# deepalcoholic/mlcomp

Hardware: AMD Instinct MI355X
Metric: images/sec (whole node) ResNet-50 DAG train task (higher is better)
Workload: dtype bf16; 1 GPU; model=resnet50, global_batch=512, per_gpu_batch=512, image_size=224, parallelism=dp1, impl=native, optimizer=SGD momentum 0.9, wd 5e-5, fp32 master weights

## Files before the change

mlcomp_amd/ops/_lib.py:

```python
from __future__ import annotations

import ctypes as C
import os
import threading

import torch

_LIB = None
_LOCK = threading.Lock()

DETERMINISTIC = os.environ.get('MLC_DETERMINISTIC', '0') == '1'
DET_COPIES = max(32, int(os.environ.get('MLC_DET_COPIES', '4096')))

vp, i32, i64, f32, u32 = C.c_void_p, C.c_int, C.c_long, C.c_float, C.c_uint

_SIGS = {
    'mlc_conv_fwd': [vp, vp, vp, vp, vp] + [i32] * 12 + [vp, vp, vp],
    'mlc_conv_fwd_ld': [vp, vp, vp] + [i32] * 13 + [vp],
    'mlc_conv_dgrad': [vp] * 4 + [i32] * 12 + [vp] * 11 + [vp],
    'mlc_conv_dgrad_t': [vp] * 4 + [i32] * 12 + [vp] * 11 + [vp],
    'mlc_bilinear_up_fwd': [vp, vp] + [i32] * 6 + [vp],
    'mlc_bilinear_up_bwd': [vp, vp] + [i32] * 6 + [vp],
    'mlc_gn_relu_fwd': [vp, vp, vp, vp, vp] + [i32] * 4 + [f32, vp],
    'mlc_gn_relu_bwd': [vp] * 7 + [i32] * 4 + [f32, vp],
    'mlc_conv_tr_fwd': [vp] * 5 + [i32] * 12 + [vp],
    'mlc_wt_transpose': [vp, i32, i64, vp],
    'mlc_conv_wgrad': [vp, vp, vp] + [i32] * 14 + [vp, i64, vp, vp, vp],
    'mlc_conv_wgrad_native': [vp, vp, vp] + [i32] * 14 + [vp, i64, vp, vp, vp],
    'mlc_gemm_f32out': [vp, vp, vp, vp] + [i32] * 11 + [vp],
    'mlc_gemm_bf16out': [vp, vp, vp] + [i32] * 8 + [vp],
    'mlc_gemm256_nt': [vp, vp, vp, vp] + [i32] * 6 + [vp, i32, vp, vp, i32, i32, vp],
    'mlc_g256_dense': [vp, vp, vp] + [i32] * 7 + [vp, i32, vp, vp, vp, i32, vp],
    'mlc_gemm256_tn': [vp, vp, vp] + [i32] * 8 + [vp],
    'mlc_conv256_fwd': [vp] * 5 + [i32] * 13 + [vp],
    'mlc_augment': [vp, vp, vp, vp] + [i32] * 7 + [vp],
    'mlc_gemm_bf16_ex': [vp, vp, vp] + [i32] * 8 + [vp, i32, vp, vp, vp, vp, i64, vp],
    'mlc_gemm_bf16_ex_native': [vp, vp, vp] + [i32] * 8 + [vp, i32, vp, vp, vp, vp, i64, vp],
    'mlc_ln_fwd': [vp] * 8 + [i32, i32, f32, f32, f32, vp, u32, u32, vp],
    'mlc_ln_bwd': [vp] * 10 + [i32, i32, f32, f32, vp, u32, u32, vp],
    'mlc_ln_finalize_many': [vp, i32, i32, vp],
    'mlc_embed_bwd': [vp] * 7 + [i32] * 4 + [vp],
    'mlc_softmax_fwd': [vp] * 4 + [i64, i32, i32, f32, f32, vp, u32, vp],
    'mlc_softmax_bwd': [vp] * 3 + [i64, i32, f32, f32, vp, u32, vp],
    'mlc_linear_wgrad_bias': [vp] * 4 + [i32] * 7 + [vp, i64, vp],
    'mlc_linear_wgrad_bias_native': [vp] * 4 + [i32] * 7 + [vp, i64, vp],
    'mlc_blaslt_mode': [i32],
    'mlc_blaslt_choices': [vp, i32],
    'mlc_upcat_fwd': [vp, vp, vp] + [i32] * 5 + [vp],
    'mlc_upcat_bwd': [vp, vp, vp] + [i32] * 5 + [vp],
    'mlc_seg_head_fwd': [vp] * 6 + [i64, i32, i32, vp],
    'mlc_seg_head_bwd': [vp] * 8 + [i64, i32, i32, f32, f32, f32, vp],
    'mlc_attn_fwd': [vp] * 4 + [i32, i32, i32, f32, f32, vp, u32, vp],
    'mlc_attn_bwd': [vp] * 5 + [i32, i32, i32, f32, f32, vp, u32, vp],
    'mlc_flash_fwd': [vp] * 4 + [i32] * 4 + [f32, f32, vp, u32, vp],
    'mlc_flash_bwd': [vp] * 7 + [i32] * 4 + [f32, f32, vp, u32, vp],
    'mlc_flash_fwd_masked': [vp] * 4 + [i32] * 4 + [f32, f32, vp, u32, i32, vp, i64, i64, vp],
    'mlc_flash_bwd_masked': [vp] * 7 + [i32] * 4 + [f32, f32, vp, u32, i32, vp, i64, i64, vp],
    'mlc_flash_bwd128': [i32],
    'mlc_colsum_acc': [vp, vp, vp, i32, i32, vp],
    'mlc_dropout': [vp, vp, i64, f32, vp, u32, vp],
    'mlc_bn_stat_copies': [],
    'mlc_set_deterministic': [i32, i32],
    'mlc_get_stat_copies': [],
    'mlc_get_deterministic': [],
    'mlc_gemm_config': [i32],
    'mlc_gemm_get_set': [i32, i32],
    'mlc_bn_get_set': [i32, i32],
    'mlc_bn_finalize': [vp, vp, i32] + [vp] * 8 + [i64, i32, f32, f32, vp],
    'mlc_bn_fwd_apply': [vp] * 5 + [i64, i32, i32, vp],
    'mlc_bn_fwd_apply2': [vp] * 7 + [i64, i32, i32, vp],
    'mlc_bn_bwd_reduce': [vp] * 5 + [i64, i32, vp],
    'mlc_bn_bwd_finalize': [vp] * 6 + [i64, i32, vp],
    'mlc_bn_fwd_fused': [vp] * 5 + [i32] + [vp] * 10 + [i64, i32, f32, f32, i32, vp],
    'mlc_bn_bwd_fused': [vp] * 5 + [i32] + [vp] * 6 + [i64, i32, vp],
    'mlc_bnact_fused': [vp] * 5 + [i32] + [vp] * 10 + [i64, i32, f32, f32, i32, f32, vp, i64, vp, i32, vp, i64, vp],
    'mlc_bn_bwd_apply': [vp] * 7 + [i64, i32, vp],
    'mlc_conv1x1_bn_bwd': [vp] * 18 + [i64, i32, i32, vp],
    'mlc_conv1x1_bn_bwd_ok': [i32, i32],
    'mlc_conv1x1_bwd_get_set': [i32, i32],
    'mlc_maxpool_fwd': [vp, vp, vp] + [i32] * 9 + [vp],
    'mlc_maxpool_bwd': [vp, vp, vp] + [i32] * 9 + [vp],
    'mlc_stem_pool_fwd': [vp] * 6 + [i32] * 4 + [vp],
    'mlc_stem_pool_bwd_reduce_pooled': [vp] * 5 + [i32] * 4 + [vp],
    'mlc_stem_pool_bwd_reduce': [vp] * 5 + [i32] * 4 + [vp],
    'mlc_stem_pool_bwd_apply': [vp] * 6 + [i32] * 4 + [vp],
    'mlc_stem_s2d': [vp, vp] + [i32] * 5 + [vp],
    'mlc_stem_conv_fwd': [vp] * 5 + [i32] * 3 + [vp],
    'mlc_avgpool_fwd': [vp, vp, i32, i32, i32, vp],
    'mlc_avgpool_bwd': [vp, vp, vp, i32, i32, i32, vp],
    'mlc_avgpool2d_fwd': [vp, vp] + [i32] * 10 + [vp],
    'mlc_avgpool2d_bwd': [vp, vp, vp] + [i32] * 10 + [vp],
    'mlc_adaptive_avg_fwd': [vp, vp] + [i32] * 6 + [vp],
    'mlc_adaptive_avg_bwd': [vp, vp] + [i32] * 6 + [vp],
    'mlc_softmax_ce': [vp] * 5 + [i32, i32, i32, f32, f32, vp],
    'mlc_colsum': [vp, vp, i32, i32, vp],
    'mlc_nchw_to_nhwc': [vp, vp, i32, i32, i32, i32, vp],
    'mlc_cast_f32_bf16': [vp, vp, i64, vp],
    'mlc_sgd': [vp] * 5 + [i64, i64, i64, f32, f32, f32, i32, i32, vp],
    'mlc_adam': [vp] * 6 + [i64, i64, i64, f32, f32, f32, f32, i32, vp],
    'mlc_sqnorm': [vp, i64, vp, f32, vp],
    'mlc_opt_config': [i32, i32],
    'mlc_gconv_wb_elems': [i32] * 6,
    'mlc_gconv_fwd': [vp] * 6 + [i32] * 13 + [vp],
    'mlc_gconv_dgrad': [vp] * 4 + [i32] * 13 + [vp],
    'mlc_gconv_wgrad': [vp] * 3 + [i32] * 14 + [vp],
    'mlc_dwconv_fwd': [vp] * 5 + [i32] * 11 + [vp],
    'mlc_dwconv_dgrad': [vp] * 3 + [i32] * 11 + [vp],
    'mlc_dwconv_wgrad': [vp] * 4 + [i32] * 12 + [vp],
    'mlc_bn_stats': [vp, vp, vp, i64, i32, vp],
    'mlc_zero4': [vp, i64, vp, i64, vp, i64, vp, i64, vp],
    'mlc_bn_stats_ld': [vp, vp, vp, i64, i32, i32, i64, vp],
    'mlc_bnact_apply': [vp] * 7 + [i64, i32, i32, f32, vp, i64, vp],
    'mlc_bnact_bwd_reduce': [vp] * 10 + [i64, i32, i32, f32, vp, i64, i64, vp],
    'mlc_bnact_bwd': [vp] * 12 + [i64] + [vp] * 5 + [i64, i32, i32, f32, vp, i64, vp, i64, i64, vp, i32, vp],
    'mlc_bnact_bwd_apply': [vp] * 12 + [i64, i32, i32, f32, vp, i64, vp, i64, i64, vp, i32, vp],
    'mlc_act_fwd': [vp, vp, i64, i32, f32, vp],
    'mlc_act_bwd': [vp] * 4 + [i64, i32, f32, vp],
    'mlc_chscale_fwd': [vp] * 4 + [i32, i64, i32, i32, vp],
    'mlc_chscale_bwd': [vp] * 8 + [i32] * 3 + [vp],
    'mlc_conv_fwd_ex': [vp] * 4 + [i32] * 13 + [vp],
    'mlc_conv_wgrad_bias': [vp] * 4 + [i32] * 13 + [vp, i64, vp],
    'mlc_temporal_unfold': [vp, vp] + [i32] * 9 + [vp],
    'mlc_temporal_fold': [vp, vp, vp] + [i32] * 9 + [vp],
    'mlc_counters_owner': [i32],
    'mlc_counters_release': [i32],
    'mlc_counters_in_use': [],
    'mlc_comm_unique_id_bytes': [],
    'mlc_comm_get_unique_id': [vp],
    'mlc_comm_init': [vp, i32, i32, i32, i32, vp],
    'mlc_comm_async_error': [vp],
    'mlc_comm_abort': [vp],
    'mlc_comm_error_string': [i32],
    'mlc_comm_last_error': [vp],
    'mlc_comm_set_timeout': [i64],
    'mlc_comm_destroy': [vp],
    'mlc_allreduce': [vp, vp, vp, i64, i32, i32, vp],
    'mlc_broadcast': [vp, vp, vp, i64, i32, i32, vp],
    'mlc_reduce_scatter': [vp, vp, vp, i64, i32, i32, vp],
    'mlc_allgather': [vp, vp, vp, i64, i32, vp],
    'mlc_alltoall': [vp, vp, vp, i64, i32, i32, i32, vp],
}
_RESTYPE = {'mlc_comm_init': vp, 'mlc_gconv_wb_elems': C.c_long, 'mlc_counters_owner': None,
            'mlc_counters_release': C.c_long, 'mlc_counters_in_use': C.c_long,
            'mlc_comm_error_string': C.c_char_p, 'mlc_comm_last_error': C.c_char_p, 'mlc_comm_set_timeout': None}


def lib_path():
    from mlcomp_amd.build import KERNEL_LIB
    return os.environ.get('MLC_KERNEL_LIB') or KERNEL_LIB


def load():
    global _LIB
    if _LIB is not None:
        return _LIB
    with _LOCK:
        if _LIB is not None:
            return _LIB
        path = lib_path()
        if not os.path.exists(path):
            from mlcomp_amd.build import build_kernels
            build_kernels()
        lib = C.CDLL(path)
        for name, args in _SIGS.items():
            fn = getattr(lib, name)
            fn.argtypes = args
            fn.restype = _RESTYPE.get(name, C.c_int)
        for key, env in ((1, 'MLC_SPLIT_TARGET'), (2, 'MLC_SPLIT_TARGET_MAT'), (3, 'MLC_GEMM_BIG'),
                         (4, 'MLC_GEMM_BIG_MIN'), (5, 'MLC_GEMM_SINGLE_STAGE'), (6, 'MLC_SPLITK_FUSED'),
                         (9, 'MLC_SPLIT_TARGET_DENSE'), (12, 'MLC_DENSE_SPLIT_TARGET'), (13, 'MLC_SINGLE_STAGE_KT'),
                         (15, 'MLC_GEMM_PERSIST_NBUF'), (16, 'MLC_GEMM_PERSIST_KT')):
            if os.environ.get(env):
                lib.mlc_gemm_get_set(key, int(os.environ[env]))
        for key, env in ((0, 'MLC_BN_UNROLL'), (1, 'MLC_BN_BLOCKS')):
            if os.environ.get(env):
                lib.mlc_bn_get_set(key, int(os.environ[env]))
        if os.environ.get('MLC_FUSE_1X1_BLOCKS'):
            lib.mlc_conv1x1_bwd_get_set(0, int(os.environ['MLC_FUSE_1X1_BLOCKS']))
        if DETERMINISTIC:
            lib.mlc_set_deterministic(1, DET_COPIES)
            torch.use_deterministic_algorithms(True, warn_only=True)
        _LIB = lib
    return _LIB


def available() -> bool:
    return torch.cuda.is_available()


def stream():
    return C.c_void_p(torch.cuda.current_stream().cuda_stream)


def ptr(t):
    if t is None:
        return None
    return C.c_void_p(t.data_ptr())


def call(name, *args):
    rc = getattr(load(), name)(*args)
    if rc == -2 and DETERMINISTIC:
        raise RuntimeError(f'{name}: deterministic mode needs more partial-sum copies than '
                           f'MLC_DET_COPIES={DET_COPIES} (one per contributing block; raise it)')
    if rc != 0:
        raise RuntimeError(f'{name} failed (rc={rc}); check shape constraints '
                           f'(channels % 8 == 0) or HIP error')
    return rc
```

mlcomp_amd/ops/functional.py:

```python
from __future__ import annotations

from typing import Optional, Tuple

import contextlib
import math
import os
import threading

import torch
import torch.nn.functional as F

from . import _lib


def _cuda(t):
    return t is not None and t.is_cuda


def conv_out_hw(H, W, KH, KW, stride, pad, dil):
    ph, pw = (pad, pad) if isinstance(pad, int) else tuple(pad)
    Ho = (H + 2 * ph - dil * (KH - 1) - 1) // stride + 1
    Wo = (W + 2 * pw - dil * (KW - 1) - 1) // stride + 1
    return Ho, Wo


def pack_pad(pad) -> int:
    if isinstance(pad, int):
        return pad
    ph, pw = (int(v) for v in pad)
    return ph if ph == pw else (1 << 30) | (pw << 15) | ph


def bn_relu_input(x: torch.Tensor, in_affine) -> torch.Tensor:
    sc, sh = in_affine
    return torch.relu(x.float() * sc + sh).to(torch.bfloat16)


def conv2d_fwd(x: torch.Tensor, w: torch.Tensor, stride=1, pad=0, dil=1,
               stats: Optional[Tuple[torch.Tensor, torch.Tensor]] = None,
               out: Optional[torch.Tensor] = None, in_affine=None) -> torch.Tensor:
    N, H, W, C = x.shape
    Co, KH, KW, Ci = w.shape
    assert Ci == C, (w.shape, x.shape)
    Ho, Wo = conv_out_hw(H, W, KH, KW, stride, pad, dil)
    if _cuda(x):
        y = out if out is not None else torch.empty(N, Ho, Wo, Co, device=x.device, dtype=torch.bfloat16)
        ldy = rows_ld(y)
        if ldy != Co:
            assert ldy is not None and stats is None and in_affine is None, (y.shape, y.stride())
            _lib.call('mlc_conv_fwd_ld', _lib.ptr(x), _lib.ptr(w), _lib.ptr(y), ldy, N, H, W, C, Co, KH, KW, stride,
                      pack_pad(pad), dil, Ho, Wo, _lib.stream())
            return y
        s1, s2 = (stats if stats is not None else (None, None))
        sc, sh = in_affine if in_affine is not None else (None, None)
        _lib.call('mlc_conv_fwd', _lib.ptr(x), _lib.ptr(w), _lib.ptr(y), _lib.ptr(s1), _lib.ptr(s2),
                  N, H, W, C, Co, KH, KW, stride, pack_pad(pad), dil, Ho, Wo, _lib.ptr(sc), _lib.ptr(sh), _lib.stream())
        return y
    if in_affine is not None:
        x = bn_relu_input(x, in_affine)
    yf = F.conv2d(x.permute(0, 3, 1, 2).float(), w.permute(0, 3, 1, 2).float(), None, stride, pad, dil)
    if stats is not None:
        stats[0][:Co].add_(yf.sum(dim=(0, 2, 3)))
        stats[1][:Co].add_((yf * yf).sum(dim=(0, 2, 3)))
    y = yf.permute(0, 2, 3, 1).to(torch.bfloat16).contiguous()
    if out is not None:
        out.copy_(y)
        return out
    return y


def conv_transpose2d_fwd(x: torch.Tensor, w: torch.Tensor, out_hw, stride=2, pad=1, dil=1,
                         stats: Optional[Tuple[torch.Tensor, torch.Tensor]] = None) -> torch.Tensor:
    N, Hi, Wi, Cin = x.shape
    Cw, KH, KW, Cout = w.shape
    assert Cw == Cin, (w.shape, x.shape)
    Ho, Wo = out_hw
    assert conv_out_hw(Ho, Wo, KH, KW, stride, pad, dil) == (Hi, Wi), (out_hw, x.shape)
    if _cuda(x):
        y = torch.empty(N, Ho, Wo, Cout, device=x.device, dtype=torch.bfloat16)
        s1, s2 = (stats if stats is not None else (None, None))
        _lib.call('mlc_conv_tr_fwd', _lib.ptr(x), _lib.ptr(w), _lib.ptr(y), _lib.ptr(s1), _lib.ptr(s2),
                  N, Hi, Wi, Cin, Cout, KH, KW, stride, pack_pad(pad), dil, Ho, Wo, _lib.stream())
        return y
    oph = Ho - ((Hi - 1) * stride - 2 * pad + dil * (KH - 1) + 1)
    opw = Wo - ((Wi - 1) * stride - 2 * pad + dil * (KW - 1) + 1)
    yf = F.conv_transpose2d(x.permute(0, 3, 1, 2).float(), w.permute(0, 3, 1, 2).float(), None, stride, pad,
                            (oph, opw), 1, dil)
    if stats is not None:
        stats[0][:Cout].add_(yf.sum(dim=(0, 2, 3)))
        stats[1][:Cout].add_((yf * yf).sum(dim=(0, 2, 3)))
    return yf.permute(0, 2, 3, 1).to(torch.bfloat16).contiguous()


class BnBwdSpec:

    def __init__(self, mask, ys, affine=None):
        assert 1 <= len(ys) <= 2
        assert affine is None or (mask is None and len(affine) == len(ys))
        self.mask = mask
        self.ys = list(ys)
        self.affine = list(affine) if affine is not None else None


def wt_flip_transpose(w: torch.Tensor) -> torch.Tensor:
    return w.flip(1, 2).permute(3, 1, 2, 0).contiguous()


def dgrad_as_fwd_conv(KH, KW, stride, pad, dil) -> bool:
    return stride == 1 and pad <= dil * (KH - 1) and dil * (KH - 1) - pad == dil * (KW - 1) - pad


class WtTable:

    def __init__(self):
        self.slots = []
        self.views = []
        self.buf = None
        self.desc = None
        self.blocks = 0
        self._srcs = None

    def add(self, slot) -> int:
        self.slots.append(slot)
        return len(self.slots) - 1

    def __getitem__(self, i) -> torch.Tensor:
        return self.views[i]

    @staticmethod
    def _dims(shape):
        return tuple(shape) if len(shape) == 4 else (shape[0], 1, 1, shape[1])

    def finalize(self, device):
        if not self.slots:
            return
        total = sum((s.numel + 63) // 64 * 64 for s in self.slots)
        self.buf = torch.zeros(total, device=device, dtype=torch.bfloat16)
        off = 0
        for s in self.slots:
            Co, KH, KW, Ci = self._dims(s.shape)
            v = self.buf[off:off + s.numel]
            self.views.append(v.view(Ci, KH, KW, Co) if len(s.shape) == 4 else v.view(Ci, Co))
            off += (s.numel + 63) // 64 * 64
        if self.buf.is_cuda:
            self._build()

    def _build(self):
        rows, blk = [], 0
        for s, v in zip(self.slots, self.views):
            Co, KH, KW, Ci = self._dims(s.shape)
            rows.append([s.bf16.data_ptr(), v.data_ptr(), Co, KH * KW, Ci, blk])
            blk += KH * KW * ((Co + 63) // 64) * ((Ci + 63) // 64)
        self.desc = torch.tensor(rows, dtype=torch.int64).to(self.buf.device)
        self.blocks = blk
        self._srcs = [r[0] for r in rows]

    def refresh(self):
        if self.buf is None:
            return
        if not self.buf.is_cuda:
            for s, v in zip(self.slots, self.views):
                v.copy_(wt_flip_transpose(s.bf16) if s.bf16.dim() == 4 else s.bf16.t())
            return
        if self._srcs != [s.bf16.data_ptr() for s in self.slots]:
            self._build()
        _lib.call('mlc_wt_transpose', _lib.ptr(self.desc), len(self.slots), self.blocks, _lib.stream())


def conv2d_dgrad(dy: torch.Tensor, w: torch.Tensor, x_shape, stride=1, pad=0, dil=1,
                 addend: Optional[torch.Tensor] = None, out: Optional[torch.Tensor] = None,
                 bn: Optional[BnBwdSpec] = None, wt: Optional[torch.Tensor] = None) -> torch.Tensor:
    N, H, W, C = x_shape
    Co, KH, KW, Ci = w.shape
    _, Ho, Wo, _ = dy.shape
    if _cuda(dy):
        dx = out if out is not None else torch.empty(N, H, W, C, device=dy.device, dtype=torch.bfloat16)
        b = [None] * 11
        if bn is not None:
            b[0] = bn.mask
            for k, (yk, mk, sk) in enumerate(bn.ys):
                b[1 + 3 * k:4 + 3 * k] = [yk, mk, sk]
            for k, (ak, hk) in enumerate(bn.affine or []):
                b[7 + 2 * k:9 + 2 * k] = [ak, hk]
        if wt is not None:
            assert tuple(wt.shape) == (Ci, KH, KW, Co), (wt.shape, w.shape)
            _lib.call('mlc_conv_dgrad_t', _lib.ptr(dy), _lib.ptr(wt), _lib.ptr(dx), _lib.ptr(addend), N, H, W,
                      C, Co, KH, KW, stride, pack_pad(pad), dil, Ho, Wo, *[_lib.ptr(t) for t in b], _lib.stream())
            return dx
        _lib.call('mlc_conv_dgrad', _lib.ptr(dy), _lib.ptr(w), _lib.ptr(dx), _lib.ptr(addend), N, H, W, C,
                  Co, KH, KW, stride, pack_pad(pad), dil, Ho, Wo, *[_lib.ptr(t) for t in b], _lib.stream())
        return dx
    if wt is not None and isinstance(pad, int) and dgrad_as_fwd_conv(KH, KW, stride, pad, dil):
        dxf = F.conv2d(dy.permute(0, 3, 1, 2).float(), wt.permute(0, 3, 1, 2).float(), None, 1,
                       dil * (KH - 1) - pad, dil)
    else:
        if wt is not None:
            w = wt_flip_transpose(wt)
        dxf = torch.nn.grad.conv2d_input((N, C, H, W), w.permute(0, 3, 1, 2).float(),
                                         dy.permute(0, 3, 1, 2).float(), stride, pad, dil)
    dxf = dxf.permute(0, 2, 3, 1)
    if addend is not None:
        dxf = dxf + addend.float()
    if bn is not None:
        if bn.mask is not None:
            dxf = dxf * (bn.mask.float() > 0)
        elif bn.affine is not None:
            q = sum(yk.float() * ak + hk for (yk, _, _), (ak, hk) in zip(bn.ys, bn.affine))
            dxf = dxf * (q > 0)
        d = dxf.to(torch.bfloat16).float().reshape(-1, C)
        for yk, mk, sk in bn.ys:
            sv = sk.view(NSTAT, 2, C)
            sv[0, 0] += d.sum(0)
            sv[0, 1] += (d * (yk.float().reshape(-1, C) - mk)).sum(0)
    dx = dxf.to(torch.bfloat16).contiguous()
    if out is not None:
        out.copy_(dx)
        return out
    return dx


_USE_SLAB = os.environ.get('MLC_WGRAD_SLAB', '1') != '0'
_SLAB = {}
_SLAB_OLD = []


_ROLE = threading.local()


def register_side_stream(stream) -> None:
    """Kept for callers of the old API: the workspace role is now explicit (side_role)."""


@contextlib.contextmanager
def side_stream(stream):
    prev = getattr(_ROLE, 'side', False)
    _ROLE.side = True
    try:
        with torch.cuda.stream(stream):
            yield
    finally:
        _ROLE.side = prev


class CounterLease:
    _next = 0

    def __init__(self, device):
        CounterLease._next += 1
        self.owner = CounterLease._next
        self.device = torch.device(device)

    def release(self):
        if self.owner and torch.cuda.is_available():
            from . import _lib
            with torch.cuda.device(self.device):
                _lib.load().mlc_counters_release(self.owner)
        self.owner = 0

    def __del__(self):
        try:
            self.release()
        except Exception:
            pass


@contextlib.contextmanager
def capture_scope(store: dict):
    prev = getattr(_ROLE, 'capture', None)
    _ROLE.capture = store
    lease = None
    if torch.cuda.is_available():
        from . import _lib
        lease = store.setdefault('__counter_lease__', CounterLease(torch.cuda.current_device()))
        _lib.load().mlc_counters_owner(lease.owner)
    try:
        yield
    finally:
        _ROLE.capture = prev
        if lease is not None:
            _lib.load().mlc_counters_owner(0)


def workspace_key(device) -> str:
    device = torch.device(device)
    if device.type == 'cuda' and getattr(_ROLE, 'side', False):
        return f'{device}/side'
    return str(device)


def workspace_store(pool: dict) -> dict:
    cap = getattr(_ROLE, 'capture', None)
    if cap is not None and torch.cuda.is_available() and torch.cuda.is_current_stream_capturing():
        return cap.setdefault(id(pool), {})
    return pool


def slab_workspace(device, n: int) -> torch.Tensor:
    key = workspace_key(device)
    store = workspace_store(_SLAB)
    buf = store.get(key)
    if buf is None or buf.numel() < n:
        if buf is not None:
            _SLAB_OLD.append(buf)
        buf = torch.empty(max(n, 1 << 20), device=device, dtype=torch.float32)
        store[key] = buf
    return buf


def conv2d_wgrad(dy: torch.Tensor, x: torch.Tensor, w_shape, stride=1, pad=0, dil=1,
                 out: Optional[torch.Tensor] = None, accumulate=False, in_affine=None,
                 slab: Optional[bool] = None) -> torch.Tensor:
    Co, KH, KW, Ci = w_shape
    N, H, W, C = x.shape
    _, Ho, Wo, _ = dy.shape
    if _cuda(dy):
        dw = out if out is not None else torch.empty(Co, KH, KW, Ci, device=dy.device, dtype=torch.float32)
        use = _USE_SLAB if slab is None else slab
        ws = slab_workspace(dy.device, min(32 * Co * KH * KW * Ci, 64 << 20)) if use else None
        sc, sh = in_affine if in_affine is not None else (None, None)
        _lib.call('mlc_conv_wgrad', _lib.ptr(dy), _lib.ptr(x), _lib.ptr(dw), N, H, W, C, Co, KH, KW,
                  stride, pack_pad(pad), dil, Ho, Wo, 0, int(accumulate), _lib.ptr(ws),
                  ws.numel() if ws is not None else 0, _lib.ptr(sc), _lib.ptr(sh), _lib.stream())
        return dw
    if in_affine is not None:
        x = bn_relu_input(x, in_affine)
    dwf = torch.nn.grad.conv2d_weight(x.permute(0, 3, 1, 2).float(), (Co, Ci, KH, KW),
                                      dy.permute(0, 3, 1, 2).float(), stride, pad, dil)
    dwf = dwf.permute(0, 2, 3, 1)
    if out is not None:
        if accumulate:
            out.add_(dwf.reshape(out.shape))
        else:
            out.copy_(dwf.reshape(out.shape))
        return out
    return dwf.contiguous()


NSTAT = _lib.DET_COPIES if _lib.DETERMINISTIC else 32


def stat_buffers(C, device):
    b = torch.zeros(2, NSTAT * C, device=device, dtype=torch.float32)
    return b[0], b[1]


BN_FUSED = os.environ.get('MLC_BN_FUSED', '1') == '1'


def _bn_fused_ok(C, ncopy):
    return BN_FUSED and not _lib.DETERMINISTIC and C % 8 == 0 and C >= 8 and 1 <= ncopy <= 64


def bn_fwd_apply(y, res, s1, s2, gamma, beta, save_mean, save_invstd, run_mean, run_var,
                 eps=1e-5, momentum=0.1, relu=True, out=None, scale=None, shift=None,
                 res_affine=None, apply=True):
    rows = y.numel() // y.shape[-1]
    C = y.shape[-1]
    ncopy = s1.numel() // C
    if _cuda(y):
        if scale is None:
            scale = torch.empty(2, C, device=y.device, dtype=torch.float32)
            scale, shift = scale[0], scale[1]
        if apply and _bn_fused_ok(C, ncopy):
            z = out if out is not None else torch.empty_like(y)
            rs, rh = res_affine if res_affine is not None else (None, None)
            _lib.call('mlc_bn_fwd_fused', _lib.ptr(y), _lib.ptr(res), _lib.ptr(z), _lib.ptr(s1), _lib.ptr(s2), ncopy,
                      _lib.ptr(gamma), _lib.ptr(beta), _lib.ptr(save_mean), _lib.ptr(save_invstd), _lib.ptr(scale),
                      _lib.ptr(shift), _lib.ptr(run_mean), _lib.ptr(run_var), _lib.ptr(rs), _lib.ptr(rh), rows, C,
                      float(eps), float(momentum), int(relu), _lib.stream())
            return z
# ... 1025 lines not shown
```

mlcomp_amd/ops/layers.py:

```python
from __future__ import annotations

import os
from typing import List, Optional

import torch
import torch.nn as nn

from . import functional as Fn
from .arena import ParamArena, Slot

DGRAD_FIRST_ENV = os.environ.get('MLC_DGRAD_FIRST')


class Workspace:

    def __init__(self):
        self._req: List[tuple] = []
        self.buf = None
        self.views = {}

    def request(self, key, n):
        self._req.append((key, int(n)))
        return key

    def finalize(self, device):
        total = sum((n + 63) // 64 * 64 for _, n in self._req) or 64
        self.buf = torch.zeros(total, device=device, dtype=torch.float32)
        off = 0
        for key, n in self._req:
            self.views[key] = self.buf[off:off + n]
            off += (n + 63) // 64 * 64

    def __getitem__(self, key):
        return self.views[key]

    def zero(self):
        self.buf.zero_()


class NativeContext:

    def __init__(self):
        self.arena = ParamArena()
        self.ws = Workspace()
        self.anchor = None
        self.training = True
        self.device = None
        self.grad_prezeroed = False
        self.wgrad_stream = None
        self.wt = Fn.WtTable() if os.environ.get('MLC_DGRAD_WT', '1') == '1' else None
        self.wt_stale = False
        self.wgrad_lag = int(os.environ.get('MLC_WGRAD_LAG', '0') or 0)
        self.wgrad_defer = False
        self._pending_wgrad = []
        self.dgrad_first = DGRAD_FIRST_ENV == '1'
        self.wgrad_slab = os.environ.get('MLC_WGRAD_SLAB', '1') != '0'

    def default_wgrad_slab(self, on: bool):
        if os.environ.get('MLC_WGRAD_SLAB') is None:
            self.wgrad_slab = on

    def default_dgrad_first(self, on: bool):
        if DGRAD_FIRST_ENV is None:
            self.dgrad_first = on

    def finalize(self, device):
        self.device = torch.device(device)
        self.arena.finalize(device)
        self.ws.finalize(device)
        if self.wt is not None:
            self.wt.finalize(self.device)
        self.anchor = torch.zeros(1, device=device, requires_grad=True)
        self.arena.flush = self.flush_wgrad
        if self.device.type == 'cuda' and os.environ.get('MLC_WGRAD_STREAM', '1') in ('1', '2'):
            self.wgrad_stream = torch.cuda.Stream(self.device)
        self.default_wgrad_defer(False)

    def default_wgrad_defer(self, on: bool):
        env = os.environ.get('MLC_WGRAD_DEFER')
        self.wgrad_defer = (env == '1') if env is not None else on
        self.arena.grad_streams = [self.wgrad_stream] if (self.wgrad_defer and self.wgrad_stream) else []

    def flush_wgrad(self):
        if self.wgrad_defer and self.wgrad_stream is not None:
            cur = torch.cuda.current_stream(self.device)
            if cur != self.wgrad_stream:
                cur.wait_stream(self.wgrad_stream)
        self.join_wgrads(0)

    def default_wgrad_lag(self, n: int):
        if os.environ.get('MLC_WGRAD_LAG') is None:
            self.wgrad_lag = n

    def lag_wgrad(self, ev, keep, slots):
        self._pending_wgrad.append((ev, keep, slots))
        self.join_wgrads(self.wgrad_lag)

    def join_wgrads(self, keep_last: int):
        q = self._pending_wgrad
        while len(q) > keep_last:
            ev, _keep, slots = q.pop(0)
            cur = torch.cuda.current_stream(self.device)
            if cur != self.wgrad_stream:
                cur.wait_event(ev)
            for s in (slots if isinstance(slots, (list, tuple)) else (slots,)):
                self.arena.mark_ready(s)

    def refresh_wt(self):
        if self.wt is not None and self.training:
            self.wt.refresh()
        self.wt_stale = False


def flatten_bn_buffers(units) -> Optional[torch.Tensor]:
    units = [u for u in units if getattr(u, 'run_mean', None) is not None]
    if not units:
        return None
    flat = torch.empty(sum(2 * u.run_mean.numel() for u in units), device=units[0].run_mean.device)
    off = 0
    for u in units:
        C = u.run_mean.numel()
        flat[off:off + C].copy_(u.run_mean)
        flat[off + C:off + 2 * C].copy_(u.run_var)
        u.run_mean, u.run_var = flat[off:off + C], flat[off + C:off + 2 * C]
        off += 2 * C
    return flat


class ConvBN:

    def __init__(self, ctx: NativeContext, name: str, conv: nn.Conv2d, bn: nn.BatchNorm2d,
                 act: bool, cin_pad: Optional[int] = None, s2d: bool = False):
        assert conv.groups == 1, 'native ConvBN supports groups=1'
        self.ctx = ctx
        self.name = name
        Co, Ci, KH, KW = conv.weight.shape
        self.cin = Ci
        self.cin_p = cin_pad or Ci
        self.Co = Co
        self.k = (KH, KW)
        self.stride = conv.stride[0]
        self.pad = conv.padding[0]
        self.dil = conv.dilation[0]
        self.s2d = s2d
        if s2d:
            assert (KH, KW, self.stride, self.pad, self.dil) == (7, 7, 2, 3, 1) and Ci <= 3, \
                's2d stem needs a 7x7/2 pad-3 conv over <= 3 channels'
            self.k, self.stride, self.pad, self.cin_p = (4, 4), 1, 0, 16
            KH = KW = 4
        self.act = act
        self.eps = bn.eps
        self.momentum = bn.momentum if bn.momentum is not None else 0.1
        self.w = ctx.arena.weight(f'{name}.conv.weight', (Co, KH, KW, self.cin_p))
        self.wt_idx = None
        if ctx.wt is not None and not s2d:
            self.wt_idx = ctx.wt.add(self.w)
        self.gamma = ctx.arena.vector(f'{name}.bn.weight', (Co,))
        self.beta = ctx.arena.vector(f'{name}.bn.bias', (Co,))
        self._src = (conv, bn)
        self.k_s1 = ctx.ws.request(f'{name}.s1', Fn.NSTAT * Co)
        self.k_s2 = ctx.ws.request(f'{name}.s2', Fn.NSTAT * Co)
        self.k_bw = ctx.ws.request(f'{name}.bwd', Fn.NSTAT * 2 * Co)

    def load_from_torch(self):
        conv, bn = self._src
        dev = self.ctx.device
        if self.s2d:
            w = Fn.stem_w_to_s2d(conv.weight.detach().cpu())
            self._gmask = (Fn.stem_w_to_s2d(torch.ones(self.Co, self.cin, 7, 7)) != 0).float().to(dev)
        else:
            w = conv.weight.detach().permute(0, 2, 3, 1).float()
            if self.cin_p != self.cin:
                w = torch.nn.functional.pad(w, (0, self.cin_p - self.cin))
        self.w.master.copy_(w.to(dev))
        self.gamma.master.copy_(bn.weight.detach().to(dev))
        self.beta.master.copy_(bn.bias.detach().to(dev))
        self.run_mean = bn.running_mean.detach().clone().float().to(dev)
        self.run_var = bn.running_var.detach().clone().float().to(dev)
        Co = self.Co
        b = torch.zeros(7, Co, device=dev)
        self.save_mean, self.save_invstd, self.scale, self.shift = b[0], b[1], b[2], b[3]
        self.coef = b[4:7].reshape(-1)

    def export_to_torch(self):
        conv, bn = self._src
        if self.s2d:
            w = Fn.stem_w_from_s2d(self.w.master.detach().float().cpu(), self.cin)
        else:
            w = self.w.master[..., :self.cin].permute(0, 3, 1, 2).contiguous()
        conv.weight.data.copy_(w.to(conv.weight.device))
        bn.weight.data.copy_(self.gamma.master.to(bn.weight.device))
        bn.bias.data.copy_(self.beta.master.to(bn.bias.device))
        bn.running_mean.copy_(self.run_mean.to(bn.running_mean.device))
        bn.running_var.copy_(self.run_var.to(bn.running_var.device))

    def __call__(self, x, res=None):
        return _ConvBNFn.apply(x, res, self.ctx.anchor, self)

    def fwd(self, x, res=None, defer=False, in_affine=None):
        ws = self.ctx.ws
        if self.s2d and x.shape[-1] != 16:
            x = Fn.stem_s2d(x, 3)
        raff = None
        if isinstance(res, tuple):
            res, rs, rh = res
            raff = (rs, rh)
        if not self.ctx.training:
            y = self._conv(x, None, in_affine)
            torch.rsqrt(self.run_var + self.eps, out=self.scale).mul_(self.gamma.master)
            torch.sub(self.beta.master, self.run_mean * self.scale, out=self.shift)
            if defer:
                return None, (x, y, None)
            z = Fn.bn_apply(y, res, self.scale, self.shift, self.act, res_affine=raff)
            return z, (x, y, z)
        s1, s2 = ws[self.k_s1], ws[self.k_s2]
        self.ctx.wt_stale = True
        y = self._conv(x, (s1, s2), in_affine)
        training = self.ctx.training
        z = Fn.bn_fwd_apply(y, res, s1, s2, self.gamma.master, self.beta.master, self.save_mean,
                            self.save_invstd, self.run_mean if training else None,
                            self.run_var if training else None, self.eps, self.momentum, self.act,
                            scale=self.scale, shift=self.shift, res_affine=raff, apply=not defer)
        return z, (x, y, z)

    def _conv(self, x, stats, in_affine=None):
        if self.s2d and in_affine is None:
            return Fn.stem_conv_fwd(x, self.w.bf16, stats=stats)
        return Fn.conv2d_fwd(x, self.w.bf16, self.stride, self.pad, self.dil, stats=stats, in_affine=in_affine)

    def _dgrad(self, dy, x_shape, addend=None, out=None, bn=None):
        wt = None
        if self.wt_idx is not None:
            if self.ctx.wt_stale:
                raise RuntimeError('transposed filters are stale: the model must call '
                                   'ctx.refresh_wt() after its training forward pass')
            wt = self.ctx.wt[self.wt_idx]
        return Fn.conv2d_dgrad(dy, self.w.bf16, x_shape, self.stride, self.pad, self.dil,
                               addend=addend, out=out, bn=bn, wt=wt)

    def dgrad_covers_all(self) -> bool:
        return True

    def bn_target(self, rec):
        x, y, z = rec
        return (y, self.save_mean, self.ctx.ws[self.k_bw])

    def wgrad(self, dy, x, in_affine=None):
        Fn.conv2d_wgrad(dy, x, self.w.shape, self.stride, self.pad, self.dil, out=self.w.grad,
                        accumulate=self.ctx.grad_prezeroed, in_affine=in_affine, slab=self.ctx.wgrad_slab)
        if self.s2d:
            self.w.grad.mul_(self._gmask)

    def _fused_1x1_bwd_ok(self, dz, x, dgrad_bn) -> bool:
        if not (Fn.FUSE_1X1_BWD and dz.is_cuda and type(self) is ConvBN and not self.s2d):
            return False
        if self.k != (1, 1) or self.stride != 1 or self.pad != 0 or x.shape[-1] != self.cin_p:
            return False
        if dgrad_bn is not None and (dgrad_bn.mask is not None or len(dgrad_bn.ys) != 1
                                     or dgrad_bn.affine is None):
            return False
        return Fn.conv1x1_bn_bwd_available(self.cin_p, self.Co)

    def bwd(self, dz, rec, want_dres=False, dx_addend=None, need_dx=True, dx_out=None,
            prereduced=False, dgrad_bn=None, in_affine=None, defer: Optional[list] = None):
        x, y, z = rec
        arena = self.ctx.arena
        if need_dx and prereduced and in_affine is None and self._fused_1x1_bwd_ok(dz, x, dgrad_bn):
            if not self.ctx.grad_prezeroed:
                self.w.grad.zero_()
            dx = Fn.conv1x1_bn_bwd(dz, y, x, self.w.bf16, self.save_mean, self.save_invstd,
                                   self.gamma.master, self.ctx.ws[self.k_bw], self.gamma.grad,
                                   self.beta.grad, self.w.grad, addend=dx_addend, out=dx_out, bn=dgrad_bn)
            arena.mark_ready(self.gamma)
            arena.mark_ready(self.beta)
            arena.mark_ready(self.w)
            return dx, (dz if want_dres else None)
        dy, dres = Fn.bn_bwd(dz, z if self.act else None, y, self.save_mean, self.save_invstd,
                             self.gamma.master, want_dres=want_dres, dgamma=self.gamma.grad,
                             dbeta=self.beta.grad, sums=self.ctx.ws[self.k_bw], zero_sums=False,
                             coef=self.coef, prereduced=prereduced)
        arena.mark_ready(self.gamma)
        arena.mark_ready(self.beta)
        side = self.ctx.wgrad_stream if need_dx else None
        if side is not None and torch.cuda.current_stream(self.ctx.device) == side:
            side = None
        fork = None
        if side is not None:
            main = torch.cuda.current_stream(self.ctx.device)
            fork = torch.cuda.Event()
            fork.record(main)
            if not self.ctx.dgrad_first:
                side.wait_event(fork)
                with Fn.side_stream(side):
                    self.wgrad(dy, x, in_affine)
        else:
            self.wgrad(dy, x, in_affine)
        dx = None
        if need_dx:
            dx = self._dgrad(dy, x.shape, addend=dx_addend, out=dx_out, bn=dgrad_bn)
        if side is not None and self.ctx.dgrad_first:
            side.wait_event(fork)
            with Fn.side_stream(side):
                self.wgrad(dy, x, in_affine)
        if side is not None and defer is not None:
            defer.append((dy, x, self.w))
            return dx, dres
        if side is not None and self.ctx.wgrad_defer:
            dy.record_stream(side)
            x.record_stream(side)
            arena.mark_ready(self.w)
            return dx, dres
        if side is not None and self.ctx.wgrad_lag:
            ev = torch.cuda.Event()
            ev.record(side)
            self.ctx.lag_wgrad(ev, (dy, x), self.w)
            return dx, dres
        if side is not None:
            main.wait_stream(side)
        arena.mark_ready(self.w)
        return dx, dres


class ConvTBN(ConvBN):

    def __init__(self, ctx: NativeContext, name: str, conv: nn.ConvTranspose2d, bn: nn.BatchNorm2d, act: bool):
        assert conv.groups == 1 and conv.dilation[0] == conv.dilation[1], 'native ConvTBN: groups=1'
        assert conv.stride[0] == conv.stride[1] and conv.padding[0] == conv.padding[1]
        self.ctx = ctx
        self.name = name
        Cin, Cout, KH, KW = conv.weight.shape
        assert bn.num_features == Cout
        self.cin = self.cin_p = Cout
        self.Co = Cout
        self.k = (KH, KW)
        self.stride, self.pad, self.dil = conv.stride[0], conv.padding[0], conv.dilation[0]
        self.out_pad = conv.output_padding
        self.s2d = False
        self.act = act
        self.eps = bn.eps
        self.momentum = bn.momentum if bn.momentum is not None else 0.1
        self.w = ctx.arena.weight(f'{name}.conv.weight', (Cin, KH, KW, Cout))
        self.wt_idx = None
        self.gamma = ctx.arena.vector(f'{name}.bn.weight', (Cout,))
        self.beta = ctx.arena.vector(f'{name}.bn.bias', (Cout,))
        self._src = (conv, bn)
        self.k_s1 = ctx.ws.request(f'{name}.s1', Fn.NSTAT * Cout)
        self.k_s2 = ctx.ws.request(f'{name}.s2', Fn.NSTAT * Cout)
        self.k_bw = ctx.ws.request(f'{name}.bwd', Fn.NSTAT * 2 * Cout)

    def _bias(self):
        conv = self._src[0]
        return conv.bias.detach().float().to(self.ctx.device) if conv.bias is not None else None

    def load_from_torch(self):
        super().load_from_torch()
        b = self._bias()
        if b is not None:
            self.run_mean.sub_(b)

    def export_to_torch(self):
        super().export_to_torch()
        b = self._bias()
        if b is not None:
            bn = self._src[1]
            bn.running_mean.add_(b.to(bn.running_mean.device))

    def out_hw(self, H, W):
        KH, KW = self.k
        return ((H - 1) * self.stride - 2 * self.pad + self.dil * (KH - 1) + self.out_pad[0] + 1,
                (W - 1) * self.stride - 2 * self.pad + self.dil * (KW - 1) + self.out_pad[1] + 1)

    def _conv(self, x, stats, in_affine=None):
        assert in_affine is None
        return Fn.conv_transpose2d_fwd(x, self.w.bf16, self.out_hw(x.shape[1], x.shape[2]), self.stride,
                                       self.pad, self.dil, stats=stats)

    def _dgrad(self, dy, x_shape, addend=None, out=None, bn=None):
        assert addend is None and out is None and bn is None, 'ConvTBN input gradient: plain conv'
        dx = Fn.conv2d_fwd(dy, self.w.bf16, self.stride, self.pad, self.dil)
        assert tuple(dx.shape) == tuple(x_shape), (dx.shape, x_shape)
        return dx

    def wgrad(self, dy, x, in_affine=None):
        assert in_affine is None
        Fn.conv2d_wgrad(x, dy, self.w.shape, self.stride, self.pad, self.dil, out=self.w.grad,
                        accumulate=self.ctx.grad_prezeroed)


class _ConvBNFn(torch.autograd.Function):
    @staticmethod
    def forward(ctx, x, res, anchor, m: ConvBN):
        z, rec = m.fwd(x, res)
        ctx.m = m
        ctx.has_res = res is not None
        ctx.save_for_backward(*rec)
        return z

    @staticmethod
    def backward(ctx, dz):
        m: ConvBN = ctx.m
        dx, dres = m.bwd(dz.contiguous(), ctx.saved_tensors, want_dres=ctx.has_res,
                         need_dx=ctx.needs_input_grad[0])
        return dx, dres, None, None


class ResidualBlock:

    def __init__(self, units: List[ConvBN], down: Optional[ConvBN]):
        self.units = units
        self.down = down
        self.ctx = units[0].ctx
        self.prev: Optional['ResidualBlock'] = None
        self.fuse_bn_bwd = True
        self.down_stream = os.environ.get('MLC_DOWN_STREAM', '1') == '1'
        mode = int(os.environ.get('MLC_FUSE_BN_FWD', '0'))
        one = lambda u: u.k == (1, 1) and u.stride == 1 and u.pad == 0
        self.fuse_into = [False] + [
            mode >= 1 and prev.act and (mode == 2 or (one(u) and (mode != 3 or u.cin <= 64)))
            for prev, u in zip(units[:-1], units[1:])]
        self.dout_prereduced = False
        self._last = None

    @property
    def fuse_bn_fwd(self) -> bool:
        return any(self.fuse_into)

    @fuse_bn_fwd.setter
    def fuse_bn_fwd(self, on: bool):
        self.fuse_into = [False] + [bool(on) and p.act for p in self.units[:-1]]

    def in_affines(self):
        return [None] + [(p.scale, p.shift) if f else None for p, f in zip(self.units[:-1], self.fuse_into[1:])]

    def __call__(self, x):
        return _ResidualBlockFn.apply(x, self.ctx.anchor, self)

    def output_bn_spec(self):
        rec, rd = self._last
        last = self.units[-1]
        ys = [last.bn_target(rec)]
        if self.down is not None and not self.down.act:
            ys.append(self.down.bn_target(rd))
            return Fn.BnBwdSpec(None, ys, affine=[(last.scale, last.shift),
                                                  (self.down.scale, self.down.shift)])
        if self.down is not None:
            ys.append(self.down.bn_target(rd))
        return Fn.BnBwdSpec(rec[2], ys)


class _ResidualBlockFn(torch.autograd.Function):
    @staticmethod
    def forward(ctx, x, anchor, blk: ResidualBlock):
        recs = []
        side = blk.ctx.wgrad_stream if (blk.down is not None and blk.down_stream) else None
        if side is not None:
            main = torch.cuda.current_stream(blk.ctx.device)
            side.wait_stream(main)
        if blk.down is not None:
            if side is not None:
                with Fn.side_stream(side):
                    _, rd = blk.down.fwd(x, defer=not blk.down.act)
            else:
                _, rd = blk.down.fwd(x, defer=not blk.down.act)
            identity = rd[2] if blk.down.act else (rd[1], blk.down.scale, blk.down.shift)
        else:
            identity, rd = x, None
        y = x
        affs = blk.in_affines()
        for i, u in enumerate(blk.units[:-1]):
            if blk.fuse_into[i + 1]:
                _, r = u.fwd(y, defer=True, in_affine=affs[i])
                y = r[1]
            else:
                y, r = u.fwd(y, in_affine=affs[i])
            recs.append(r)
        if side is not None:
            main.wait_stream(side)
        out, r = blk.units[-1].fwd(y, identity, in_affine=affs[-1])
        recs.append(r)
        blk._last = (r, rd)
        ctx.blk = blk
        ctx.n = len(recs)
        flat = [t for r in recs for t in r]
        if rd is not None:
            flat += list(rd)
        ctx.save_for_backward(*flat)
        return out

    @staticmethod
    def backward(ctx, dout):
        blk: ResidualBlock = ctx.blk
        saved = ctx.saved_tensors
        recs = [saved[3 * i:3 * i + 3] for i in range(ctx.n)]
        rd = saved[3 * ctx.n:3 * ctx.n + 3] if blk.down is not None else None
        dout = dout.contiguous()
        need_dx = ctx.needs_input_grad[0]
        pre = blk.dout_prereduced
        blk.dout_prereduced = False
        units = blk.units
        fuse = blk.fuse_bn_bwd
        affs = blk.in_affines()
        if blk.fuse_bn_fwd:
            assert fuse, 'the BN-apply fusion needs the fused BN-backward reductions (z is not stored)'

        def spec_for(i):
            u = units[i]
            if not fuse or not units[i + 1].dgrad_covers_all():
                return None
            if u.act:
                return Fn.BnBwdSpec(None, [u.bn_target(recs[i])], affine=[(u.scale, u.shift)])
            return Fn.BnBwdSpec(None, [u.bn_target(recs[i])])

        side = units[0].ctx.wgrad_stream
        pend = [] if side is not None and os.environ.get('MLC_WGRAD_STREAM') == '2' else None
        sp = spec_for(len(units) - 2) if len(units) > 1 else None
        d, dres = units[-1].bwd(dout, recs[-1], want_dres=True, prereduced=pre, dgrad_bn=sp,
                                in_affine=affs[-1], defer=pend)
        fused = sp is not None
        down_side = side if (blk.down is not None and pend is None and blk.down_stream) else None
        short = dres
        if down_side is not None:
            main = torch.cuda.current_stream(units[0].ctx.device)
            short_buf = torch.empty(rd[0].shape, device=rd[0].device, dtype=rd[0].dtype) if need_dx else None
            down_side.wait_stream(main)
            with Fn.side_stream(down_side):
                short, _ = blk.down.bwd(dres, rd, need_dx=need_dx, prereduced=pre, dx_out=short_buf)
        for i in range(len(units) - 2, 0, -1):
            sp = spec_for(i - 1)
            d, _ = units[i].bwd(d, recs[i], prereduced=fused, dgrad_bn=sp, in_affine=affs[i], defer=pend)
            fused = sp is not None
        if down_side is not None:
# ... 147 lines not shown
```

Before: 14160 images/s.

## Add persistent 1x1 conv forward kernel with register-resident weights and fused BN stats

```diff
diff --git a/csrc/kernels/conv1x1_fwd.hip b/csrc/kernels/conv1x1_fwd.hip
--- /dev/null
+++ b/csrc/kernels/conv1x1_fwd.hip
@@ -0,0 +1,208 @@
+#include "common.h"
+
+namespace {
+
+constexpr int NT = 256;
+constexpr int BM = 64;
+constexpr int CHUNK = 256;
+
+typedef __amdgpu_buffer_rsrc_t Rsrc;
+constexpr unsigned OOB = 0x80000000u;
+__device__ __forceinline__ Rsrc rsrc(const void* base, long bytes) {
+  return __builtin_amdgcn_make_buffer_rsrc(const_cast<void*>(base), (short)0,
+                                           (int)(bytes < 0x7ffffff0L ? bytes : 0x7ffffff0L), 0x00020000);
+}
+__device__ __forceinline__ uint4 bload(Rsrc r, unsigned voff) {
+  return __builtin_bit_cast(uint4, __builtin_amdgcn_raw_buffer_load_b128(r, voff, 0, 0));
+}
+__device__ __forceinline__ void bstore(Rsrc r, unsigned voff, int imm, const uint4& v) {
+  typedef unsigned u32x4 __attribute__((ext_vector_type(4)));
+  __builtin_amdgcn_raw_buffer_store_b128(u32x4{v.x, v.y, v.z, v.w}, r, voff, imm, 0);
+}
+__device__ __forceinline__ void lds_barrier() { asm volatile("s_waitcnt lgkmcnt(0)\n\ts_barrier" ::: "memory"); }
+
+struct FwdArgs {
+  const bf16* x; const bf16* w; bf16* y; float* sum; float* sumsq;
+  long rows; int Co; int groups; int ncopy;
+};
+
+template <int K>
+__global__ void __launch_bounds__(NT, 1) conv1x1_fwd_kernel(const FwdArgs a) {
+  constexpr int LD = K + 8;
+  constexpr int KS = K / 16;
+  constexpr int CPR = K / 8;
+  constexpr int RPI = NT / CPR;
+  constexpr int CPT = BM / RPI;
+  static_assert(NT % CPR == 0 && BM % RPI == 0, "x tile staging");
+  __shared__ __attribute__((aligned(16))) bf16 sX[2][BM * LD];
+
+  const int t = threadIdx.x, lane = t & 63, wv = t >> 6, l32 = lane & 31, h = lane >> 5;
+  const long rows = a.rows;
+  const int ntiles = (int)((rows + BM - 1) / BM);
+  const int G = a.groups, nch = a.Co / CHUNK;
+  int rg, chunk;
+  if ((G & 7) == 0) {
+    const int q = blockIdx.x >> 3;
+    chunk = q % nch;
+    rg = (q / nch) * 8 + (blockIdx.x & 7);
+  } else {
+    chunk = blockIdx.x % nch;
+    rg = blockIdx.x / nch;
+  }
+  if (rg >= ntiles) return;
+  const int cb = chunk * CHUNK + wv * 64;
+
+  bf16x8 wf[2][KS];
+#pragma unroll
+  for (int i = 0; i < 2; ++i)
+#pragma unroll
+    for (int s = 0; s < KS; ++s)
+      wf[i][s] = __builtin_bit_cast(bf16x8, ldg16(a.w + (long)(cb + 32 * i + l32) * K + s * 16 + h * 8));
+
+  f32x16 s1[2], s2[2];
+#pragma unroll
+  for (int i = 0; i < 2; ++i)
+#pragma unroll
+    for (int r = 0; r < 16; ++r) { s1[i][r] = 0.f; s2[i][r] = 0.f; }
+
+  const int xc = t % CPR, xr0 = t / CPR;
+  uint4 xv[CPT];
+  auto rows_left = [&](int tile) {
+    const long left = rows - (long)tile * BM;
+    return (int)(left < 0 ? 0 : left > BM ? BM : left);
+  };
+  unsigned xoff[CPT];
+#pragma unroll
+  for (int u = 0; u < CPT; ++u) xoff[u] = (unsigned)((xr0 + RPI * u) * K + xc * 8) * 2u;
+  auto prefetch = [&](int tile) {
+    const int left = rows_left(tile);
+    const long m0 = left > 0 ? (long)tile * BM : 0;
+    const Rsrc rs = rsrc(a.x + m0 * K, (rows - m0) * K * 2);
+#pragma unroll
+    for (int u = 0; u < CPT; ++u) xv[u] = bload(rs, xr0 + RPI * u < left ? xoff[u] : OOB);
+  };
+
+  auto stage = [&](int buf) {
+#pragma unroll
+    for (int u = 0; u < CPT; ++u) *reinterpret_cast<uint4*>(sX[buf] + (xr0 + RPI * u) * LD + xc * 8) = xv[u];
+  };
+
+  int tile = rg, buf = 0;
+  __builtin_amdgcn_s_waitcnt(0x0f70);
+  __builtin_amdgcn_sched_barrier(0);
+  prefetch(tile);
+  stage(0);
+  prefetch(tile + G);
+#pragma unroll 1
+  for (; tile < ntiles; tile += G, buf ^= 1) {
+    const long m0 = (long)tile * BM;
+    const bf16* sx = sX[buf];
+    lds_barrier();
+
+    f32x16 acc[2][2];
+#pragma unroll
+    for (int i = 0; i < 2; ++i)
+#pragma unroll
+      for (int j = 0; j < 2; ++j)
+#pragma unroll
+        for (int r = 0; r < 16; ++r) acc[i][j][r] = 0.f;
+#pragma unroll
+    for (int s = 0; s < KS; ++s) {
+      bf16x8 xf[2];
+#pragma unroll
+      for (int j = 0; j < 2; ++j)
+        xf[j] = *reinterpret_cast<const bf16x8*>(sx + (32 * j + l32) * LD + s * 16 + h * 8);
+#pragma unroll
+      for (int i = 0; i < 2; ++i)
+#pragma unroll
+        for (int j = 0; j < 2; ++j)
+          acc[i][j] = __builtin_amdgcn_mfma_f32_32x32x16_bf16(wf[i][s], xf[j], acc[i][j], 0, 0, 0);
+    }
+
+    const Rsrc ys = rsrc(a.y + m0 * a.Co, (rows - m0) * a.Co * 2);
+    const int left = rows_left(tile);
+#pragma unroll
+    for (int j = 0; j < 2; ++j) {
+      const unsigned yoff = 32 * j + l32 < left ? (unsigned)((32 * j + l32) * a.Co + cb + 8 * h) * 2u : OOB;
+#pragma unroll
+      for (int i = 0; i < 2; ++i) {
+#pragma unroll
+        for (int r = 0; r < 16; ++r) {
+          const float v = acc[i][j][r];
+          s1[i][r] += v;
+          s2[i][r] += v * v;
+        }
+#pragma unroll
+        for (int q = 0; q < 4; q += 2) {
+          uint32_t a0 = pack2_bf16(acc[i][j][4 * q], acc[i][j][4 * q + 1]);
+          uint32_t a1 = pack2_bf16(acc[i][j][4 * q + 2], acc[i][j][4 * q + 3]);
+          uint32_t b0 = pack2_bf16(acc[i][j][4 * q + 4], acc[i][j][4 * q + 5]);
+          uint32_t b1 = pack2_bf16(acc[i][j][4 * q + 6], acc[i][j][4 * q + 7]);
+          const auto e0 = __builtin_amdgcn_permlane32_swap(a0, b0, false, false);
+          const auto e1 = __builtin_amdgcn_permlane32_swap(a1, b1, false, false);
+          bstore(ys, yoff, (32 * i + 8 * q) * 2, make_uint4(e0[0], e1[0], e0[1], e1[1]));
+        }
+      }
+    }
+    __builtin_amdgcn_sched_barrier(0);
+    stage(buf ^ 1);
+    prefetch(tile + 2 * G);
+  }
+
+  float* d1 = a.sum + (size_t)((unsigned)rg % (unsigned)a.ncopy) * a.Co;
+  float* d2 = a.sumsq + (size_t)((unsigned)rg % (unsigned)a.ncopy) * a.Co;
+#pragma unroll
+  for (int i = 0; i < 2; ++i)
+#pragma unroll
+    for (int r = 0; r < 16; ++r) {
+      float u = s1[i][r], v = s2[i][r];
+#pragma unroll
+      for (int o = 16; o > 0; o >>= 1) { u += __shfl_xor(u, o, 64); v += __shfl_xor(v, o, 64); }
+      if (l32 == 0) {
+        const int c = cb + 32 * i + (r & 3) + 8 * (r >> 2) + 4 * h;
+        atomicAdd(d1 + c, u);
+        atomicAdd(d2 + c, v);
+      }
+    }
+}
+
+int g_fwd_max_blocks = 0;
+
+int cu_count() {
+  static int n = 0;
+  if (!n) {
+    int dev = 0;
+    hipDeviceProp_t p;
+    if (hipGetDevice(&dev) != hipSuccess || hipGetDeviceProperties(&p, dev) != hipSuccess) return 256;
+    n = p.multiProcessorCount > 0 ? p.multiProcessorCount : 256;
+  }
+  return n;
+}
+
+}
+
+MLC_EXPORT int mlc_conv1x1_fwd_ok(int Cin, int Cout) {
+  return !g_mlc_det && ((Cin == 128 && Cout == 512) || (Cin == 256 && Cout == 1024));
+}
+
+MLC_EXPORT int mlc_conv1x1_fwd_get_set(int key, int value) {
+  if (key != 0) return -1;
+  const int old = g_fwd_max_blocks;
+  if (value >= 0) g_fwd_max_blocks = value;
+  return old;
+}
+
+MLC_EXPORT int mlc_conv1x1_fwd(const bf16* x, const bf16* w, bf16* y, float* sum, float* sumsq, long rows,
+                               int Cin, int Cout, hipStream_t st) {
+  if (!mlc_conv1x1_fwd_ok(Cin, Cout) || !sum || !sumsq || rows < 1 || rows > (1L << 36)) return -1;
+  const int nch = Cout / CHUNK;
+  const long ntiles = (rows + BM - 1) / BM;
+  long groups = (g_fwd_max_blocks > 0 ? g_fwd_max_blocks : cu_count()) / nch;
+  if (groups > ntiles) groups = ntiles;
+  if (groups < 1) groups = 1;
+  const FwdArgs a{x, w, y, sum, sumsq, rows, Cout, (int)groups, g_mlc_ncopy};
+  const dim3 grid((unsigned)(groups * nch));
+  if (Cin == 128) hipLaunchKernelGGL((conv1x1_fwd_kernel<128>), grid, dim3(NT), 0, st, a);
+  else hipLaunchKernelGGL((conv1x1_fwd_kernel<256>), grid, dim3(NT), 0, st, a);
+  return hipGetLastError();
+}
diff --git a/mlcomp_amd/ops/_lib.py b/mlcomp_amd/ops/_lib.py
--- a/mlcomp_amd/ops/_lib.py
+++ b/mlcomp_amd/ops/_lib.py
@@ -78,6 +78,9 @@
     'mlc_conv1x1_bn_bwd': [vp] * 18 + [i64, i32, i32, vp],
     'mlc_conv1x1_bn_bwd_ok': [i32, i32],
     'mlc_conv1x1_bwd_get_set': [i32, i32],
+    'mlc_conv1x1_fwd': [vp] * 5 + [i64, i32, i32, vp],
+    'mlc_conv1x1_fwd_ok': [i32, i32],
+    'mlc_conv1x1_fwd_get_set': [i32, i32],
     'mlc_maxpool_fwd': [vp, vp, vp] + [i32] * 9 + [vp],
     'mlc_maxpool_bwd': [vp, vp, vp] + [i32] * 9 + [vp],
     'mlc_stem_pool_fwd': [vp] * 6 + [i32] * 4 + [vp],
@@ -177,6 +180,8 @@
                 lib.mlc_bn_get_set(key, int(os.environ[env]))
         if os.environ.get('MLC_FUSE_1X1_BLOCKS'):
             lib.mlc_conv1x1_bwd_get_set(0, int(os.environ['MLC_FUSE_1X1_BLOCKS']))
+        if os.environ.get('MLC_CONV1X1_FWD_BLOCKS'):
+            lib.mlc_conv1x1_fwd_get_set(0, int(os.environ['MLC_CONV1X1_FWD_BLOCKS']))
         if DETERMINISTIC:
             lib.mlc_set_deterministic(1, DET_COPIES)
             torch.use_deterministic_algorithms(True, warn_only=True)
diff --git a/mlcomp_amd/ops/functional.py b/mlcomp_amd/ops/functional.py
--- a/mlcomp_amd/ops/functional.py
+++ b/mlcomp_amd/ops/functional.py
@@ -66,6 +66,26 @@
     if out is not None:
         out.copy_(y)
         return out
+    return y
+
+
+CONV1X1_FWD = os.environ.get('MLC_CONV1X1_FWD', '1') == '1'
+
+
+def conv1x1_fwd_available(Cin, Cout) -> bool:
+    return not _lib.DETERMINISTIC and bool(_lib.load().mlc_conv1x1_fwd_ok(Cin, Cout))
+
+
+def conv1x1_fwd(x: torch.Tensor, w: torch.Tensor, stats: Tuple[torch.Tensor, torch.Tensor],
+                out: Optional[torch.Tensor] = None) -> torch.Tensor:
+    Co, KH, KW, Ci = w.shape
+    assert (KH, KW) == (1, 1) and x.shape[-1] == Ci and stats is not None, (w.shape, x.shape)
+    if not _cuda(x):
+        return conv2d_fwd(x, w, stats=stats, out=out)
+    y = out if out is not None else torch.empty(*x.shape[:-1], Co, device=x.device, dtype=torch.bfloat16)
+    assert y.is_contiguous() and x.is_contiguous(), (y.stride(), x.stride())
+    _lib.call('mlc_conv1x1_fwd', _lib.ptr(x), _lib.ptr(w), _lib.ptr(y), _lib.ptr(stats[0]), _lib.ptr(stats[1]),
+              x.numel() // Ci, Ci, Co, _lib.stream())
     return y
 
 
diff --git a/mlcomp_amd/ops/layers.py b/mlcomp_amd/ops/layers.py
--- a/mlcomp_amd/ops/layers.py
+++ b/mlcomp_amd/ops/layers.py
@@ -226,7 +226,16 @@
     def _conv(self, x, stats, in_affine=None):
         if self.s2d and in_affine is None:
             return Fn.stem_conv_fwd(x, self.w.bf16, stats=stats)
+        if stats is not None and in_affine is None and self._conv1x1_fwd_ok(x):
+            return Fn.conv1x1_fwd(x, self.w.bf16, stats)
         return Fn.conv2d_fwd(x, self.w.bf16, self.stride, self.pad, self.dil, stats=stats, in_affine=in_affine)
+
+    def _conv1x1_fwd_ok(self, x) -> bool:
+        if not (Fn.CONV1X1_FWD and x.is_cuda and type(self) is ConvBN and not self.s2d):
+            return False
+        if self.k != (1, 1) or self.stride != 1 or self.pad != 0 or x.shape[-1] != self.cin_p:
+            return False
+        return Fn.conv1x1_fwd_available(self.cin_p, self.Co)
 
     def _dgrad(self, dy, x_shape, addend=None, out=None, bn=None):
         wt = None
```

After: 14330 images/s (median of 6 runs). +1.2%, better.
